# Benny44/QPALM

Measured on AMD Instinct MI355X. Metric: QP solves/sec (batched random n=1000,m=2000); `value` = solve only, batch resident in HBM -- with qpalm_setup in the clock as the reference's run_time has it: `value_setup_plus_solve`, higher is better.
Workload: dtype f64

## Files before the change

qpalm_amd/csrc/qpalm_dense.h:

```cpp
#ifndef QPALM_DENSE_H
#define QPALM_DENSE_H
#include <type_traits>

#ifdef QPALM_EMU
#define QP_FLAG_LOAD(p) (*(volatile int *)(p))
#define QP_FLAG_STORE(p, v) (*(volatile int *)(p) = (v))
#define QP_RELEASE_AGENT() do { } while (0)
#define QP_ACQUIRE_AGENT() do { } while (0)
#define QP_DRAIN_VMEM() do { } while (0)
#define QP_SLEEP() do { } while (0)
#define QP_WAVE_SYNC() emu_wave_sync()
#define QP_LDS_VBASE(p) (p)
#define QP_SCHED_BARRIER() do { } while (0)
#define QP_SETPRIO(p) do { } while (0)
#define QP_DRAIN_LDS() do { } while (0)
#else
#define QP_FLAG_LOAD(p) __hip_atomic_load((p), __ATOMIC_RELAXED, __HIP_MEMORY_SCOPE_AGENT)
#define QP_FLAG_STORE(p, v) __hip_atomic_store((p), (v), __ATOMIC_RELAXED, __HIP_MEMORY_SCOPE_AGENT)
#define QP_RELEASE_AGENT() __builtin_amdgcn_fence(__ATOMIC_RELEASE, "agent")
#define QP_ACQUIRE_AGENT() __builtin_amdgcn_fence(__ATOMIC_ACQUIRE, "agent")
#define QP_DRAIN_VMEM() asm volatile("s_waitcnt vmcnt(0)" ::: "memory")
#define QP_SLEEP() __builtin_amdgcn_s_sleep(2)
#define QP_SETPRIO(p) __builtin_amdgcn_s_setprio(p)
#define QP_DRAIN_LDS() asm volatile("s_waitcnt lgkmcnt(0)" ::: "memory")
// ... 684 lines not shown
}

QPN void co_factor_trailing(double *L_, double *Dg_, int n, int ld, char *lds_, int J, int wg, int nwg) {
  const int NB = QP_FNB;
  if (J + NB >= n) return;
  char *stage = lds_ + ((sizeof(FactorLds) + 15) & ~(size_t)15);
  int item = 0;
  for (int Jc = J + NB; Jc < n; Jc += NB) {
    const int ntiles = (n - Jc + 15) / 16;
    for (int tbase = 0; tbase < ntiles; tbase += QP_FNT * QP_NW, item++) {
      if (item % nwg != wg) continue;
      const int rem = ntiles - tbase;
      const int ntj = (rem + QP_NW - 1) / QP_NW;
      if (ntj <= 1) factor_panel_update<1, 2>(L_, Dg_, stage, n, ld, Jc, tbase, J, J + NB);
      else factor_panel_update<2, 2>(L_, Dg_, stage, n, ld, Jc, tbase, J, J + NB);
    }
  }
}
QPN void co_factor_diag(double *L_, double *Dg_, int n, int ld, char *lds_, int J) {
  qp_gdouble *L = (qp_gdouble *)L_, *Dg = (qp_gdouble *)Dg_;
  FactorLds QP_LDS_AS &F = *QP_LDS_ARG(FactorLds, lds_);
  const int NB = QP_FNB, tid = threadIdx.x, wid = tid >> 6;
  const int jb = (n - J < NB) ? (n - J) : NB;
  __syncthreads();
  for (int e = tid; e < NB * NB; e += QP_T) {
    const int c = e / NB, r = e % NB;
    F.Ld[r][c] = (r >= c && r < jb) ? L[(size_t)(J + c) * ld + (J + r)] : ((r == c) ? 1.0 : 0.0);
  }
  __syncthreads();
  if (wid == 0) factor_diag_block(lds_);
  __syncthreads();
  for (int e = tid; e < jb * jb; e += QP_T) {
    const int c = e / jb, r = e % jb;
    if (r > c) L[(size_t)(J + c) * ld + (J + r)] = F.Ld[r][c];
  }
  if (tid < jb) Dg[J + tid] = F.dg[tid];
  __syncthreads();
}
QPN void co_factor_rows(double *L_, const double *Dg_, int n, int ld, char *lds_, int J, int wg, int nwg) {
  qp_gdouble *L = (qp_gdouble *)L_;
  const qp_gdouble *Dg = (const qp_gdouble *)Dg_;
  FactorLds QP_LDS_AS &F = *QP_LDS_ARG(FactorLds, lds_);
  constexpr int NB = QP_FNB;
  const int tid = threadIdx.x;
  const int jb = (n - J < NB) ? (n - J) : NB;
  if (J + jb >= n) return;
  __syncthreads();
  for (int e = tid; e < NB * NB; e += QP_T) {
    const int c = e / NB, r = e % NB;
    F.Ld[r][c] = (r > c && r < jb) ? L[(size_t)(J + c) * ld + (J + r)] : 0.0;
  }
  if (tid < NB) F.dv[tid] = (tid < jb) ? 1.0 / Dg[J + tid] : 1.0;
  __syncthreads();
  for (int i = J + jb + wg * QP_T + tid; i < n; i += QP_T * nwg) {
    qp_gdouble *base = L + (size_t)J * ld + i;
    double u[NB];
#pragma unroll
    for (int c = 0; c < NB; c++) u[c] = (c < jb) ? base[(size_t)c * ld] : 0.0;
#pragma unroll
    for (int c = 0; c < NB; c++) {
      if (c < jb) {
        double v = u[c];
#pragma unroll
        for (int c1 = 0; c1 < c; c1++) {
          v = QP_FMA(-u[c1], F.Ld[c][c1], v);
          if ((c1 & 7) == 7) QP_SCHED_BARRIER();
        }
        u[c] = v;
      }
      QP_SCHED_BARRIER();
    }
    int ld2 = ld;
    QP_OPAQUE(ld2);
#pragma unroll
    for (int c = 0; c < NB; c++)
      if (c < jb) base[(size_t)c * ld2] = u[c] * F.dv[c];
  }
}
#define CO_SNB 64
struct CoSolveLds {
  double tile[CO_SNB][CO_SNB + 1];
  double part[CO_SNB];
};
QPN void co_solve_forward(const double *L_, int n, int ld, double *x_, double *xo_, char *lds_, int J, int wg, int nwg) {
  const qp_gdouble *L = (const qp_gdouble *)L_;
  qp_gdouble *x = (qp_gdouble *)x_, *xo = (qp_gdouble *)xo_;
  CoSolveLds QP_LDS_AS &T = *QP_LDS_ARG(CoSolveLds, lds_);
  constexpr int NB = CO_SNB;
  const int tid = threadIdx.x, lane = tid & 63, wid = tid >> 6;
  const int jb = (n - J < NB) ? (n - J) : NB;
  __syncthreads();
  for (int e = tid; e < NB * NB; e += QP_T) {
    const int c = e / NB, r = e % NB;
    T.tile[r][c] = (r > c && r < jb) ? L[(size_t)(J + c) * ld + (J + r)] : 0.0;
  }
  __syncthreads();
  if (wid == 0) {
    double v = (lane < jb) ? x[J + lane] : 0.0;
#pragma unroll 8
    for (int c = 0; c < NB; c++) {
      const double yc = qp_readlane(v, c);
      v = QP_FMA(-T.tile[lane][c], yc, v);
    }
    T.part[lane] = v;
    if (wg == 0 && lane < jb) xo[J + lane] = v;
  }
  __syncthreads();
  for (int i = J + jb + wg * QP_T + tid; i < n; i += QP_T * nwg) {
    double acc = x[i];
#pragma unroll 1
    for (int c0 = 0; c0 < NB; c0 += 16) {
      double lv[16];
#pragma unroll
      for (int c = 0; c < 16; c++) lv[c] = QP_LDNT(3, &L[(size_t)(J + ((c0 + c < jb) ? c0 + c : jb - 1)) * ld + i]);
#pragma unroll
      for (int c = 0; c < 16; c++) if (c0 + c < jb) acc = QP_FMA(-lv[c], T.part[c0 + c], acc);
    }
    x[i] = acc;
  }
}
QPN void co_solve_backward(const double *L_, int n, int ld, double *x_, double *xo_, char *lds_, int J, int wg, int nwg) {
  const qp_gdouble *L = (const qp_gdouble *)L_;
  qp_gdouble *x = (qp_gdouble *)x_, *xo = (qp_gdouble *)xo_;
  CoSolveLds QP_LDS_AS &T = *QP_LDS_ARG(CoSolveLds, lds_);
  constexpr int NB = CO_SNB;
  const int tid = threadIdx.x, lane = tid & 63, wid = tid >> 6;
  const int jb = (n - J < NB) ? (n - J) : NB;
  __syncthreads();
  for (int e = tid; e < NB * NB; e += QP_T) {
    const int c = e / NB, r = e % NB;
    T.tile[r][c] = (r > c && r < jb) ? L[(size_t)(J + c) * ld + (J + r)] : 0.0;
  }
  __syncthreads();
  if (wid == 0) {
    double v = (lane < jb) ? x[J + lane] : 0.0;
#pragma unroll 8
    for (int r = NB - 1; r >= 0; r--) {
      const double xr = qp_readlane(v, r);
      v = QP_FMA(-T.tile[r][lane], xr, v);
    }
    T.part[lane] = (lane < jb) ? v : 0.0;
    if (wg == 0 && lane < jb) xo[J + lane] = v;
  }
  __syncthreads();
  const int grp = tid >> 4, gl = tid & 15, ngrp = QP_T / 16;
  double xb[4];
#pragma unroll
  for (int k = 0; k < 4; k++) xb[k] = T.part[4 * gl + k];
  for (int c0 = (wg * ngrp); c0 < J; c0 += ngrp * nwg) {
    const int c = c0 + grp;
    double s = 0.0;
    if (c < J) {
      const int r0 = J + 4 * gl;
      double lv[4];
#pragma unroll
      for (int k = 0; k < 4; k++) lv[k] = (r0 + k < n) ? QP_LDNT(3, &L[(size_t)c * ld + r0 + k]) : 0.0;
      s = QP_FMA(lv[1], xb[1], lv[0] * xb[0]);
      s = QP_FMA(lv[2], xb[2], s);
      s = QP_FMA(lv[3], xb[3], s);
    }
    for (int o = 8; o > 0; o >>= 1) s += __shfl_xor(s, o);
    if (c < J && gl == 0) x[c] = x[c] - s;
  }
}

#define QP_UNB 32
#ifndef QP_UNBS
#define QP_UNBS QP_UNB
#endif
#ifndef QP_UNBS32
#define QP_UNBS32 16
#endif
#ifndef QP_USQ
#define QP_USQ 1
#endif
#ifndef QP_TQD
#define QP_TQD 4
#endif
#define QP_CWG(U, buf, col) (U).cwg[buf][col]
template <int K> struct UpdownCfg {
  static constexpr int NB = (K > 16) ? QP_UNBS32 : QP_UNBS;
  static constexpr int G = (K + 15) / 16;
  static constexpr int KG = K / G;
};
template <int RPT, int K>
struct UpdownLds {
  static constexpr int NB = UpdownCfg<K>::NB;
  double Ld[2][NB][NB + 1];
  double Lsq[QP_USQ ? 2 : 1][QP_USQ ? NB : 1][NB];
  double Wd[2][NB][K + 1];
  double cwg[2][NB][K][2];
  double stash[RPT][K][64];
  double Wt[K];
  double dd[2][NB];
  double ys[2][NB];
  double stash_acc[RPT][64];
};

#ifdef QPALM_EMU
template <int N> QPD double qp_row_shr(double v) {
  const int lane = threadIdx.x & 63;
  const bool ok = (lane & 15) >= N;
  const double r = emu_exchange(v, ok ? lane - N : lane);
  return ok ? r : 0.0;
}
#else
template <int N> QPD double qp_row_shr(double v) {
  int lo = __double2loint(v), hi = __double2hiint(v);
  lo = __builtin_amdgcn_update_dpp(0, lo, 0x110 + N, 0xf, 0xf, true);
  hi = __builtin_amdgcn_update_dpp(0, hi, 0x110 + N, 0xf, 0xf, true);
  return __hiloint2double(hi, lo);
}
#endif
template <int KG> QPD double qp_rank_pivots_seq(const double p, const int ln, const double d0) {
  double run = d0 + p;
#pragma unroll
  for (int sq = 1; sq < KG; sq++) {
    const double up = qp_row_shr<1>(run);
    if ((ln & 15) == sq) run = up + p;
  }
  return run;
}
template <int KG> QPD int qp_rank_pivots(const double p, const int ln, const double d0, const int mode, double &dnew, double &dprev) {
  if (mode != QP_PIV_SEQ) {
    double incl = p;
    if (KG > 1) incl += qp_row_shr<1>(incl);
    if (KG > 2) incl += qp_row_shr<2>(incl);
    if (KG > 4) incl += qp_row_shr<4>(incl);
    if (KG > 8) incl += qp_row_shr<8>(incl);
    const double excl = qp_row_shr<1>(incl);
    dnew = d0 + incl; dprev = d0 + excl;
    if (mode == QP_PIV_TREE) return 0;
    const bool danger = !(__builtin_fabs(dnew) >= 0x1p-8 * __builtin_fabs(d0));
    if (__ballot(danger ? 1 : 0) == 0ull) return 0;
  }
  dnew = qp_rank_pivots_seq<KG>(p, ln, d0);
  const double sh = qp_row_shr<1>(dnew);
  dprev = ((ln & 15) == 0) ? d0 : sh;
  return (mode != QP_PIV_SEQ) ? 1 : 0;
}


#ifdef QPALM_EMU
template <int R> QPD double qp_row_bcast(double v) { const int lane = threadIdx.x & 63; return emu_exchange(v, (lane & ~15) | R); }
#else
template <int R> QPD double qp_row_bcast(double v) {
  return __builtin_amdgcn_update_dpp(0.0, v, 0x150 + R, 0xf, 0xf, true);
}
#endif
#ifdef QPALM_EMU
template <int K, int OFF, int R0, int R1, bool FIRST = true>
QPD void qp_apply_ranks_dpp(const double cw0, const double cw1, double (&wrow)[K], double &l) {
  const int lane = threadIdx.x & 63;
  emu_publish2(cw0, cw1);
  for (int r = R0; r < R1 && OFF + r < K; r++) {
    const double c0 = emu_peek((lane & ~15) | r, 0), c1 = emu_peek((lane & ~15) | r, 1);
    wrow[OFF + r] = QP_FMA(c0, l, wrow[OFF + r]);
    l = QP_FMA(c1, wrow[OFF + r], l);
  }
  emu_wave_sync();
}
#else
#ifndef QP_FMAC_DPP
#define QP_FMAC_DPP 1
#endif
#define QP_FD_STEP(i, n) "v_fmac_f64_dpp %" #i ", %9, %8 row_newbcast:%" #n " row_mask:0xf bank_mask:0xf bound_ctrl:1\n\t" \
                         "v_fmac_f64_dpp %8, %10, %" #i " row_newbcast:%" #n " row_mask:0xf bank_mask:0xf bound_ctrl:1\n\t"
#define QP_FD_EIGHT QP_FD_STEP(0, 11) QP_FD_STEP(1, 12) QP_FD_STEP(2, 13) QP_FD_STEP(3, 14) QP_FD_STEP(4, 15) QP_FD_STEP(5, 16) QP_FD_STEP(6, 17) QP_FD_STEP(7, 18)
template <int R0> QPD void qp_fmac_bcast8(double *w, double &l, const double cw0, const double cw1) {
  asm("s_nop 1\n\t" QP_FD_EIGHT
      : "+&v"(w[0]), "+&v"(w[1]), "+&v"(w[2]), "+&v"(w[3]), "+&v"(w[4]), "+&v"(w[5]), "+&v"(w[6]), "+&v"(w[7]), "+&v"(l)
      : "v"(cw0), "v"(cw1), "n"(R0), "n"(R0 + 1), "n"(R0 + 2), "n"(R0 + 3), "n"(R0 + 4), "n"(R0 + 5), "n"(R0 + 6), "n"(R0 + 7));
}
template <int K, int OFF, int R0, int R1, bool FIRST = true>
QPD void qp_apply_ranks_dpp(const double cw0, const double cw1, double (&wrow)[K], double &l) {
  if constexpr (QP_FMAC_DPP && R1 - R0 == 8 && OFF + R1 <= K) {
    qp_fmac_bcast8<R0>(&wrow[OFF + R0], l, cw0, cw1);
  } else if constexpr (R0 < R1 && OFF + R0 < K) {
    const double c0 = qp_row_bcast<R0>(cw0), c1 = qp_row_bcast<R0>(cw1);
    wrow[OFF + R0] = QP_FMA(c0, l, wrow[OFF + R0]);
    l = QP_FMA(c1, wrow[OFF + R0], l);
    qp_apply_ranks_dpp<K, OFF, R0 + 1, R1, false>(cw0, cw1, wrow, l);
  }
}
#endif
#ifndef QP_RECUR_DPP
#define QP_RECUR_DPP 1
#endif
#ifndef QP_AQD
#define QP_AQD 4
#endif
#ifndef QP_OWN_A
#define QP_OWN_A 1
#endif
#ifndef QP_SQ_WB
#define QP_SQ_WB 0
#endif
#ifndef QP_PANEL_A_DPP
#define QP_PANEL_A_DPP (K <= 16)
#endif
#ifndef QP_OWNER_DPP32
#define QP_OWNER_DPP32 1
#endif

template <int RPT, int K>
#ifndef QP_NI_UPDOWN
#define QP_NI_UPDOWN QPNI
#endif
QP_NI_UPDOWN void dense_updown(const int *Atp_, const int *Ati_, const double *Atss_, const int n_, const int ld_,
                               double *L_, double *Dg_, double *Wst_, const int *cols_, int n_up_,
                               const int *cols_dn_, int n_dn_, QpShared *S_, char *lds, int64_t *tdbg_, int pre_jmin_ = -1,
                               double *fs_ = nullptr, int rk0_ = 0, int rkn_ = 0x7fffffff) {
  const int n = QP_UNIFORM(n_), ld = QP_UNIFORM(ld_), n_up = QP_UNIFORM(n_up_), n_dn = QP_UNIFORM(n_dn_);
  const int rk0 = QP_UNIFORM(rk0_), rkn = QP_UNIFORM(rkn_);
  const int pre_jmin = QP_UNIFORM(pre_jmin_);
  const int pivmode = QP_UNIFORM(S_->seq_ranks);
  qp_gdouble *fs = (qp_gdouble *)fs_;
  const bool fuse_any = QP_UNIFORM((int)(fs_ != nullptr)) != 0;
  int64_t QP_LDS_AS *tdbg = (int64_t QP_LDS_AS *)tdbg_;
  const qp_gint *Atp = (const qp_gint *)Atp_, *Ati = (const qp_gint *)Ati_, *cols = (const qp_gint *)cols_, *cols_dn = (const qp_gint *)cols_dn_;
  const qp_gdouble *Atss = (const qp_gdouble *)Atss_;
  qp_gdouble *L = (qp_gdouble *)L_, *Dg = (qp_gdouble *)Dg_, *Wst = (qp_gdouble *)Wst_;
  QpShared &S = *S_;
  static_assert(K == 8 || K == 16 || K == 32, "rank groups of one DPP row (16 lanes), eight ranks at a time");
  static_assert(K <= QPG_KWST, "the staging area holds QPG_KWST dense update vectors");
  typedef UpdownLds<RPT, K> UpdownLdsT;
  UpdownLdsT QP_LDS_AS &U = *QP_LDS_ARG(UpdownLdsT, lds);
  static_assert(sizeof(UpdownLds<RPT, K>) <= ((RPT == 1) ? QP_LDS_BUDGET : QPG_LDS_DEFAULT), "update scratch must fit the dynamic LDS (the 256-thread instance only ever runs RPT = 1)");
  constexpr int NB = UpdownCfg<K>::NB, G = UpdownCfg<K>::G, KG = UpdownCfg<K>::KG;
  constexpr int PROWS = QP_T * RPT;
  constexpr bool MP = (K > 16);
  static_assert(PROWS % NB == 0, "passes start on block boundaries");
  const int lane = threadIdx.x & 63, wid = QP_UNIFORM(S.wave_rank[threadIdx.x >> 6]), tid = wid * 64 + lane;
  const int nr_all = n_up + n_dn;
  const int rk1 = (rkn < nr_all - rk0) ? (rk0 + rkn) : nr_all;
  qp_gdouble *dummy = Wst + (size_t)QPG_KWST * n;
  qp_gdouble *Tab = dummy + QPG_DUMMY + QPG_HSTASH;
  const int npass = MP ? (n + PROWS - 1) / PROWS : 1;
  for (int r0 = rk0; r0 < rk1; r0 += K) {
    const int kk = (rk1 - r0 < K) ? (rk1 - r0) : K;
    const bool fuse = fuse_any && (r0 + K >= nr_all);
    __syncthreads();
    long long tq0 = QP_CLOCK();
    int jmin = n;
    if (pre_jmin < 0) {
      for (int e = tid; e < kk * n; e += QP_T) Wst[e] = 0.0;
      __syncthreads();
      for (int r = wid; r < kk; r += QP_NW) {
        const int g = r0 + r;
        const int t = (g < n_up) ? cols[g] : cols_dn[g - n_up];
        for (int k = Atp[t] + lane; k < Atp[t + 1]; k += 64) {
          const int i = Ati[k];
          Wst[(size_t)r * n + i] = Atss[k];
          jmin = (i < jmin) ? i : jmin;
        }
      }
    } else jmin = (pre_jmin < n) ? pre_jmin : n - 1;
    if (fuse) jmin = 0;
    jmin = QP_UNIFORM(block_imin(S, jmin));
    double alpha[G], ialpha[G], sg[G];
    const int rl = QP_RECUR_DPP ? (lane & 15) : lane;
#pragma unroll
    for (int g = 0; g < G; g++) {
      alpha[g] = 1.0; ialpha[g] = 1.0;
      sg[g] = (16 * g + rl < kk) ? ((r0 + 16 * g + rl < n_up) ? 1.0 : -1.0) : 0.0;
    }
    const int J0 = (jmin / NB) * NB;
    if (tid == 0) {
      const long long tq1 = QP_CLOCK(); tdbg[0] += tq1 - tq0; tq0 = tq1;
      tdbg[QPG_CNT_SWEEPS] += 1;
      tdbg[QPG_CNT_SWEEP_ENTRIES] += (long long)(n - J0) * (n - J0 - 1) / 2 + (n - J0);
    }
    for (int pass = 0; pass < npass; pass++) {
    const int R0 = pass * PROWS;
    const int R1 = (!MP || n - R0 < PROWS) ? n : R0 + PROWS;
    const int Js = (J0 > R0) ? J0 : R0;
    if (Js >= R1) continue;
    const bool last_pass = (R1 >= n);
    const int rlim = last_pass ? ld : R1;
    if (MP && npass > 1) __syncthreads();
    double w[RPT][K];
#pragma unroll
    for (int rr = 0; rr < RPT; rr++) {
      const int i = R0 + tid * RPT + rr;
#pragma unroll
      for (int r = 0; r < K; r++) w[rr][r] = (i < R1 && r < kk) ? Wst[(size_t)r * n + i] : 0.0;
    }
    double acc[RPT];
#pragma unroll
    for (int rr = 0; rr < RPT; rr++) { const int i = R0 + tid * RPT + rr; acc[rr] = (fuse && i < R1) ? fs[i] : 0.0; }
    auto apply_table = [&](const int tb, const int Jc, const bool ok) QP_ALWAYS_INLINE {
      constexpr int QD = (K > 16) ? 2 * QP_TQD : QP_TQD;
      static_assert(NB % QD == 0, "queue depth divides the block");
      constexpr bool ODPP = QP_OWNER_DPP32 && (K > 16);
      const qp_pair QP_LDS_AS *tabO = (const qp_pair QP_LDS_AS *)QP_LDS_VBASE(&QP_CWG(U, tb, 0)[lane & 15][0]);
      const int i0 = R0 + tid * RPT;
      qp_gdouble *rowp = ok ? (L + (size_t)Jc * ld + i0) : (dummy + tid * RPT);
      const size_t cstride = ok ? (size_t)ld : 0;
      double q[QD][RPT];
#pragma unroll
      for (int cc = 0; cc < QD; cc++) qp_load_rows_nt<RPT>(rowp + (size_t)cc * cstride, q[cc]);
      auto group = [&](const int c0) QP_ALWAYS_INLINE {
#pragma unroll
        for (int u = 0; u < QD; u++) {
          int c1 = c0 + u;
          QP_OPAQUE(c1);
          double l[RPT];
          const int cpre = (c1 + QD < NB) ? c1 + QD : NB - 1;
#pragma unroll
          for (int rr = 0; rr < RPT; rr++) l[rr] = q[u][rr];
          if constexpr (ODPP) {
            qp_pair cf[G];
#pragma unroll
            for (int g = 0; g < G; g++) cf[g] = tabO[c1 * K + 16 * g];
#pragma unroll
            for (int rr = 0; rr < RPT; rr++) {
              qp_apply_ranks_dpp<K, 0, 0, 8, false>(cf[0].x, cf[0].y, w[rr], l[rr]);
              if (KG > 8 && kk > 8) qp_apply_ranks_dpp<K, 0, 8, 16, false>(cf[0].x, cf[0].y, w[rr], l[rr]);
              if constexpr (G > 1) {
                if (kk > 16) qp_apply_ranks_dpp<K, 16, 0, 8, false>(cf[G - 1].x, cf[G - 1].y, w[rr], l[rr]);
                if (kk > 24) qp_apply_ranks_dpp<K, 16, 8, 16, false>(cf[G - 1].x, cf[G - 1].y, w[rr], l[rr]);
              }
            }
          } else {
#pragma unroll
          for (int rb = 0; rb < K; rb += 4) {
            if (rb >= kk) break;
            double cf[4][2];
#pragma unroll
            for (int r = 0; r < 4; r++) {
              cf[r][0] = (rb + r < K) ? QP_CWG(U, tb, c1)[rb + r][0] : 0.0; cf[r][1] = (rb + r < K) ? QP_CWG(U, tb, c1)[rb + r][1] : 0.0;
            }
#pragma unroll
            for (int r = 0; r < 4; r++) {
              if (rb + r < K) {
#pragma unroll
                for (int rr = 0; rr < RPT; rr++) {
                  w[rr][rb + r] = QP_FMA(cf[r][0], l[rr], w[rr][rb + r]);
                  l[rr] = QP_FMA(cf[r][1], w[rr][rb + r], l[rr]);
                }
              }
            }
            QP_SCHED_BARRIER();
          }
          }
          qp_store_rows_nt<RPT>(rowp + (size_t)c1 * cstride, l);
          if (fuse) {
            const double yv = U.ys[tb][c1];
#pragma unroll
            for (int rr = 0; rr < RPT; rr++) acc[rr] = QP_FMA(-l[rr], yv, acc[rr]);
          }
          QP_SCHED_BARRIER();
          qp_load_rows_nt<RPT>(rowp + (size_t)cpre * cstride, q[u]);
          QP_SCHED_BARRIER();
        }
      };
      group(0);
#pragma unroll 1
      for (int c0 = QD; c0 < NB; c0 += QD) group(c0);
    };
    auto export_table = [&](const int tb, const int Jc, const int t0, const int nt) QP_ALWAYS_INLINE {
      const qp_pair QP_LDS_AS *src = (const qp_pair QP_LDS_AS *)&U.cwg[tb][0][0][0];
      for (int e = t0; e < NB * K; e += nt) {
        const qp_pair v = src[e];
        Tab[((size_t)Jc * K + e) * 2] = v.x; Tab[((size_t)Jc * K + e) * 2 + 1] = v.y;
      }
    };
    if constexpr (MP) if (R0 > J0) {
      const int nrb = (R0 - J0) / NB;
      const int i0 = R0 + tid * RPT;
      const bool ok = (i0 < rlim);
      constexpr int NE = (NB * K + QP_T - 1) / QP_T;
      qp_pair stg[NE];
      double ystg = 0.0;
      auto tab_load = [&](const int b) QP_ALWAYS_INLINE {
        const int Jc = J0 + b * NB;
#pragma unroll
        for (int q = 0; q < NE; q++) {
          const int e = tid + q * QP_T;
          if (e < NB * K) { stg[q].x = Tab[((size_t)Jc * K + e) * 2]; stg[q].y = Tab[((size_t)Jc * K + e) * 2 + 1]; }
        }
        if (fuse && tid < NB) ystg = fs[Jc + tid];
      };
      auto tab_store = [&](const int b) QP_ALWAYS_INLINE {
        qp_pair QP_LDS_AS *dst = (qp_pair QP_LDS_AS *)&U.cwg[b & 1][0][0][0];
#pragma unroll
        for (int q = 0; q < NE; q++) {
          const int e = tid + q * QP_T;
          if (e < NB * K) dst[e] = stg[q];
        }
        if (fuse && tid < NB) U.ys[b & 1][tid] = ystg;
      };
      tab_load(0);
      tab_store(0);
      __syncthreads();
      for (int b = 0; b < nrb; b++) {
        if (b + 1 < nrb) tab_load(b + 1);
        if (__ballot(ok ? 1 : 0) != 0ull) apply_table(b & 1, J0 + b * NB, ok);
        if (b + 1 < nrb) tab_store(b + 1);
        __syncthreads();
      }
    }
    const int nblk = (R1 - Js + NB - 1) / NB;
    {
      const int jb0 = (R1 - Js < NB) ? (R1 - Js) : NB;
#pragma unroll
      for (int rr = 0; rr < RPT; rr++) {
        const int i = R0 + tid * RPT + rr;
        if (i >= Js && i < Js + jb0) {
#pragma unroll
          for (int r = 0; r < K; r++) U.Wd[0][i - Js][r] = w[rr][r];
          U.Wd[0][i - Js][K] = acc[rr];
        }
      }
      for (int e = tid; e < jb0 * jb0; e += QP_T) {
        const int c1 = e / jb0, c = e % jb0;
        if (c > c1) U.Ld[0][c][c1] = L[(size_t)(Js + c1) * ld + (Js + c)];
      }
      if (tid < jb0) U.dd[0][tid] = Dg[Js + tid];
      if (wid == 0) {
#pragma unroll
        for (int rr = 0; rr < RPT; rr++)
#pragma unroll
          for (int r = 0; r < K; r++) U.stash[rr][r][lane] = w[rr][r];
#pragma unroll
        for (int rr = 0; rr < RPT; rr++) U.stash_acc[rr][lane] = acc[rr];
      }
    }
    if (tid == 0) { const long long tq1 = QP_CLOCK(); tdbg[0] += tq1 - tq0; tq0 = tq1; }
    __syncthreads();
    for (int s = 0; s < nblk; s++) {
      const int J = Js + s * NB, Jp = J - NB, Jn = J + NB;
      const int jb = (R1 - J < NB) ? (R1 - J) : NB;
      const int jbn = (R1 - Jn < NB) ? ((R1 - Jn > 0) ? (R1 - Jn) : 0) : NB;
      const int cur = s & 1, prv = cur ^ 1;
      long long tpe = QP_CLOCK();
      constexpr bool OWNA = QP_OWN_A && QP_USQ && !QP_SQ_WB;
      const int Ja = (OWNA && s > 0) ? J : Jn;
      const bool own_live0 = (R0 + 64 * RPT - 1 >= Ja);
      auto owner_block = [&]() QP_ALWAYS_INLINE {
        const long long tt0 = QP_CLOCK();
        bool any = false;
#pragma unroll
        for (int rr = 0; rr < RPT; rr++) { const int i = R0 + tid * RPT + rr; any = any || (i >= Ja && i < R1); }
        constexpr bool WAVES = MP && QP_OWNER_DPP32;
        if (s > 0 && (WAVES ? (__ballot(any ? 1 : 0) != 0ull) : any)) {
          const int i0 = R0 + tid * RPT;
          apply_table(prv, Jp, i0 >= Ja && i0 < rlim);
        }
#pragma unroll
        for (int rr = 0; rr < RPT; rr++) {
          const int i = R0 + tid * RPT + rr;
          if (i >= Jn && i < Jn + jbn) {
#pragma unroll
            for (int r = 0; r < K; r++) U.Wd[prv][i - Jn][r] = w[rr][r];
            U.Wd[prv][i - Jn][K] = acc[rr];
          }
        }
        if (wid == 0) {
#pragma unroll
          for (int rr = 0; rr < RPT; rr++)
#pragma unroll
            for (int r = 0; r < K; r++) U.stash[rr][r][lane] = w[rr][r];
#pragma unroll
          for (int rr = 0; rr < RPT; rr++) U.stash_acc[rr][lane] = acc[rr];
        }
        if (tid == QP_T - 64) tdbg[2] += QP_CLOCK() - tt0;
      };
      if (wid == 0) {
        const long long tp0 = QP_CLOCK();
        QP_SETPRIO(3);
        double wrow[K];
        double accp;
#pragma unroll
        for (int r = 0; r < K; r++) wrow[r] = (lane < jb) ? U.Wd[cur][lane][r] : 0.0;
        accp = (lane < jb) ? U.Wd[cur][lane][K] : 0.0;
        if (s > 0) {
          constexpr bool PSQ = QP_USQ;
          constexpr int QD = PSQ ? QP_AQD : 8;
          qp_gdouble *rowp = (lane < jb) ? (L + (size_t)Jp * ld + J + lane) : (dummy + lane);
          const size_t cstride = (lane < jb) ? (size_t)ld : 0;
          const int lrow = lane & (NB - 1);
          double q[QD];
#pragma unroll
          for (int cc = 0; cc < QD; cc++) q[cc] = PSQ ? U.Lsq[cur][cc][lrow] : rowp[(size_t)cc * cstride];
          const qp_pair QP_LDS_AS *tabA = (const qp_pair QP_LDS_AS *)QP_LDS_VBASE(&QP_CWG(U, prv, 0)[lane & 15][0]);
          qp_pair cfq[QP_PANEL_A_DPP ? QD : 1][G];
          if (QP_PANEL_A_DPP) {
#pragma unroll
            for (int cc = 0; cc < QD; cc++)
#pragma unroll
              for (int g = 0; g < G; g++) cfq[cc][g] = tabA[cc * K + 16 * g];
          }
          auto group = [&](const int c0) QP_ALWAYS_INLINE {
#pragma unroll
            for (int u = 0; u < QD; u++) {
              const int c1 = c0 + u;
              double l = q[u];
              const int cpre = (c1 + QD < NB) ? c1 + QD : NB - 1;
              if (QP_PANEL_A_DPP) {
                qp_apply_ranks_dpp<K, 0, 0, 8, false>(cfq[u][0].x, cfq[u][0].y, wrow, l);
                if (KG > 8 && kk > 8) qp_apply_ranks_dpp<K, 0, 8, 16, false>(cfq[u][0].x, cfq[u][0].y, wrow, l);
                if constexpr (G > 1) {
                  if (kk > 16) qp_apply_ranks_dpp<K, 16, 0, 8, false>(cfq[u][G - 1].x, cfq[u][G - 1].y, wrow, l);
                  if (kk > 24) qp_apply_ranks_dpp<K, 16, 8, 16, false>(cfq[u][G - 1].x, cfq[u][G - 1].y, wrow, l);
                }
              } else {
#pragma unroll
              for (int rb = 0; rb < K; rb += 8) {
                if (rb >= kk) break;
                double cw[8], cg[8];
#pragma unroll
                for (int r = 0; r < 8; r++) { cw[r] = (rb + r < K) ? QP_CWG(U, prv, c1)[rb + r][0] : 0.0; cg[r] = (rb + r < K) ? QP_CWG(U, prv, c1)[rb + r][1] : 0.0; }
#pragma unroll
                for (int r = 0; r < 8; r++) {
                  if (rb + r < K) {
                    wrow[rb + r] = QP_FMA(cw[r], l, wrow[rb + r]);
                    l = QP_FMA(cg[r], wrow[rb + r], l);
                  }
                }
                if (K > 16) QP_SCHED_BARRIER();
              }
              }
              if (PSQ && QP_SQ_WB) { if (lane < NB) U.Lsq[cur][c1][lrow] = l; }
              else if (!OWNA) rowp[(size_t)c1 * cstride] = l;
              if (fuse) accp = QP_FMA(-l, U.ys[prv][c1], accp);
              QP_SCHED_BARRIER();
              q[u] = PSQ ? U.Lsq[cur][cpre][lrow] : rowp[(size_t)cpre * cstride];
              if (QP_PANEL_A_DPP) {
#pragma unroll
                for (int g = 0; g < G; g++) cfq[u][g] = tabA[cpre * K + 16 * g];
              }
              QP_SCHED_BARRIER();
            }
          };
          group(0);
#pragma unroll 1
          for (int c0 = QD; c0 < NB; c0 += QD) group(c0);
        }
        if (QP_PANEL_TIMING == 1 && lane == 0) tdbg[8] += QP_CLOCK() - tp0;
        const long long tp1 = QP_CLOCK();
// ... 555 lines not shown
```

Baseline: 5526.

## Reorder rank-update columns by first nonzero row to shrink sweep cost

Before the low-rank update/downdate sweep, a new device routine computes each update column's first nonzero row index, then sorts the columns by that index, keeping updates ahead of downdates. It estimates a triangular sweep cost per group of K ranks for the original order and the sorted order, and rewrites the column lists in place only when the sorted order is cheaper. The aim is to group columns with late first rows so each rank group's sweep can start further down the factor and skip work. It adds an O(nr^2) rank-count sort in LDS plus several block barriers per call. It also changes the order in which updates are applied, which can alter floating-point rounding.

```diff
diff --git a/qpalm_amd/csrc/qpalm_dense.h b/qpalm_amd/csrc/qpalm_dense.h
--- a/qpalm_amd/csrc/qpalm_dense.h
+++ b/qpalm_amd/csrc/qpalm_dense.h
@@ -1010,6 +1010,77 @@
 #ifndef QP_OWNER_DPP32
 #define QP_OWNER_DPP32 1
 #endif
+
+#define QP_ORDER_MAX 512
+struct OrderLds {
+  unsigned long long key[QP_ORDER_MAX], skey[QP_ORDER_MAX];
+  int row[QP_ORDER_MAX];
+  long long cost[2][QP_ORDER_MAX / 8];
+  int keep;
+};
+template <int KC>
+QPNI void qp_order_ranks(const int *Atp_, const int *Ati_, const int n_, const int *up_, const int n_up_, const int *dn_, const int n_dn_, char *lds) {
+  const int n = QP_UNIFORM(n_), n_up = QP_UNIFORM(n_up_), n_dn = QP_UNIFORM(n_dn_);
+  const qp_gint *Atp = (const qp_gint *)Atp_, *Ati = (const qp_gint *)Ati_;
+  qp_gint *up = (qp_gint *)up_, *dn = (qp_gint *)dn_;
+  OrderLds QP_LDS_AS &O = *QP_LDS_ARG(OrderLds, lds);
+  const int nr = n_up + n_dn, tid = threadIdx.x, sub = tid & 7, grp = tid >> 3;
+  __syncthreads();
+  for (int e0 = 0; e0 < nr; e0 += QP_T / 8) {
+    const int e = e0 + grp;
+    int first = n, t = 0;
+    if (e < nr) {
+      t = (e < n_up) ? up[e] : dn[e - n_up];
+      for (int k = Atp[t] + sub; k < Atp[t + 1]; k += 8) { const int i = Ati[k]; first = (i < first) ? i : first; }
+    }
+    for (int o = 4; o > 0; o >>= 1) { const int u = __shfl_xor(first, o); first = (u < first) ? u : first; }
+    if (e < nr && sub == 0) {
+      O.key[e] = ((unsigned long long)(e >= n_up ? 1 : 0) << 62) | ((unsigned long long)(unsigned)(n - first) << 32) | (unsigned)e;
+      O.row[e] = t;
+    }
+  }
+  __syncthreads();
+  int pos[(QP_ORDER_MAX + QP_T - 1) / QP_T];
+#pragma unroll
+  for (int q = 0; q < (QP_ORDER_MAX + QP_T - 1) / QP_T; q++) {
+    const int e = tid + q * QP_T;
+    pos[q] = 0;
+    if (e < nr) {
+      const unsigned long long ke = O.key[e];
+      int c = 0;
+      for (int f = 0; f < nr; f++) c += (O.key[f] < ke) ? 1 : 0;
+      pos[q] = c;
+      O.skey[c] = ke;
+    }
+  }
+  __syncthreads();
+  const int ng = (nr + KC - 1) / KC;
+  if (tid < 2 * ng) {
+    const int which = tid / ng, g = tid - which * ng;
+    int fmin = n;
+    for (int e = KC * g; e < KC * g + KC && e < nr; e++) {
+      const int f = n - (int)(((which ? O.skey[e] : O.key[e]) >> 32) & 0x3fffffffu);
+      fmin = (f < fmin) ? f : fmin;
+    }
+    const long long c = n - ((fmin < n ? fmin : n - 1) / 32) * 32;
+    O.cost[which][g] = c * (c + 1) / 2;
+  }
+  __syncthreads();
+  if (tid == 0) {
+    long long cl = 0, cs = 0;
+    for (int g = 0; g < ng; g++) { cl += O.cost[0][g]; cs += O.cost[1][g]; }
+    O.keep = (cs < cl) ? 1 : 0;
+  }
+  __syncthreads();
+  if (O.keep) {
+#pragma unroll
+    for (int q = 0; q < (QP_ORDER_MAX + QP_T - 1) / QP_T; q++) {
+      const int e = tid + q * QP_T;
+      if (e < nr) { const int t = O.row[e]; if (pos[q] < n_up) up[pos[q]] = t; else dn[pos[q] - n_up] = t; }
+    }
+  }
+  __syncthreads();
+}
 
 template <int RPT, int K>
 #ifndef QP_NI_UPDOWN
@@ -1045,6 +1116,9 @@
   qp_gdouble *dummy = Wst + (size_t)QPG_KWST * n;
   qp_gdouble *Tab = dummy + QPG_DUMMY + QPG_HSTASH;
   const int npass = MP ? (n + PROWS - 1) / PROWS : 1;
+  static_assert(sizeof(OrderLds) <= sizeof(UpdownLdsT), "the ordering scratch fits where the sweep's LDS block will be");
+  if (rk0 == 0 && pre_jmin < 0 && nr_all > ((K < 16) ? K : 16) && nr_all <= QP_ORDER_MAX && pivmode != QP_PIV_SEQ)
+    qp_order_ranks<(K < 16) ? K : 16>(Atp_, Ati_, n, cols_, n_up, cols_dn_, n_dn, lds);
   for (int r0 = rk0; r0 < rk1; r0 += K) {
     const int kk = (rk1 - r0 < K) ? (rk1 - r0) : K;
     const bool fuse = fuse_any && (r0 + K >= nr_all);
```

After: 5754, median of 6. 1.04x the previous value.
